# skyhehe123/SA-SSD

Measured on NVIDIA H100. Metric: KITTI frames/sec (~20k pts, car_cfg voxel grid), higher is better.
Workload: dtype f32

## Files before the change

include/sassd_b200.h:

```cpp
#ifndef SASSD_B200_H
#define SASSD_B200_H

#include <stddef.h>
#include <stdint.h>

#ifdef __cplusplus
extern "C" {
#endif

typedef void* sassd_stream_t;

enum {
    SASSD_OK = 0,
    SASSD_ERR_ARG = -1,
    SASSD_ERR_LAUNCH = -2,
    SASSD_ERR_WORKSPACE = -3,
    SASSD_ERR_UNSUPPORTED = -4
};

enum {
    SASSD_FLAG_VOXEL_CAP = 1,
    SASSD_FLAG_ROWS_CAP = 2,
    SASSD_FLAG_GUIDED_CAP = 4,
    SASSD_FLAG_NMS_CAP = 8,
// ... 68 lines not shown
typedef struct {
    int32_t mode, precision;
    int32_t cin, cout, taps;
    int32_t in_stride, out_stride;
    int32_t rows_cap;
    int32_t batch, H, W;
    int32_t relu;
} sassd_gconv_desc;
int sassd_gconv(const sassd_gconv_desc* host_desc, const float* in, const float* weight, const float* scale,
                const float* shift, const int32_t* nbr, const int32_t* d_rows, float* out, sassd_stream_t stream);

size_t sassd_gconv_pack_bytes(int taps, int cin, int cout, int precision);
int sassd_gconv_pack(const float* weight, int taps, int cin, int cout, int precision, void* packed,
                     sassd_stream_t stream);

typedef struct {
    int32_t batch, H, W;
    int32_t cin, cin_stored;
    int32_t cout, taps, relu;
    int32_t out_f32_stride, out_split_ch;
    int32_t tile_order;
    int32_t n_split;
} sassd_conv2d_desc;
int sassd_conv2d_f16x3(const sassd_conv2d_desc* host_desc, const void* in_split, const void* wpack, const float* scale,
                       const float* shift, float* out_f32, void* out_split, sassd_stream_t stream);
#define SASSD_CONV2D_TILE_H 8
#define SASSD_CONV2D_TILE_W 16
#define SASSD_TILE_DIST_MAX 9
int sassd_conv2d_f16x3_occ(const sassd_conv2d_desc* host_desc, const void* in_split, const void* wpack,
                           const float* scale, const float* shift, float* out_f32, void* out_split,
// ... 126 lines not shown
```

sa-ssd_b200/csrc/conv2d_tma.cu:

```cuda
#include <cuda.h>

#include <cstdlib>

#include "tc_common.cuh"

namespace tma {

using namespace tc;

constexpr int TILE_H = SASSD_CONV2D_TILE_H, TILE_W = SASSD_CONV2D_TILE_W;
constexpr int BKC = 64;
constexpr int kConstTile = 1 << 30;
constexpr int kBgTile = 1 << 29;
constexpr int CONS_WARPS = CONS_THREADS / 32;
constexpr int THREADS2 = CONS_THREADS + 32;
constexpr int W_LOAD = CONS_WARPS;

constexpr int A_ROWS = TILE_H + 2;
constexpr int A_PLANE_BYTES = A_ROWS * TILE_W * 128;
constexpr int A_STAGE_BYTES = 2 * A_PLANE_BYTES;
constexpr int A_STAGES = 2;

template <int BN>
struct Cfg2 {
    static constexpr int B_TILE_BYTES = BN * 128;
    static constexpr int B_STAGE_BYTES = 2 * B_TILE_BYTES;
    static constexpr int B_STAGES = (BN >= 128) ? 4 : 6;
    static constexpr int RING_BYTES = A_STAGES * A_STAGE_BYTES + B_STAGES * B_STAGE_BYTES;
    static constexpr int ORDER_CAP = 4608;
    static constexpr int SMEM_BYTES = RING_BYTES + 1024 + 256 + ORDER_CAP / 4 + ORDER_CAP * 2;
    static_assert(SMEM_BYTES <= 227 * 1024, "dynamic shared memory above the sm_90 limit");
};

__device__ __forceinline__ void tma_load_4d(uint32_t dst, const CUtensorMap* map, int c0, int c1, int c2, int c3,
                                            uint32_t bar) {
    asm volatile(
        "cp.async.bulk.tensor.4d.shared::cluster.global.tile.mbarrier::complete_tx::bytes [%0], [%1, {%2, %3, %4, %5}], [%6];"
        ::"r"(dst), "l"(map), "r"(c0), "r"(c1), "r"(c2), "r"(c3), "r"(bar)
        : "memory");
}

struct Conv2dArgs {
    const void* wpack;
// ... 82 lines not shown
                                                int nthreads) {
    if (!p.out_split || c0 >= p.out_split_ch) return;
    const int vpp = (p.out_split_ch - c0) >> 3;
    const size_t plane = (size_t)p.batch * p.H * p.W * p.out_split_ch;
    const uint4 zero = make_uint4(0u, 0u, 0u, 0u);
    for (int i = tid; i < TILE_H * TILE_W * vpp; i += nthreads) {
        const int pix = i / vpp;
        const int y = ty * TILE_H + pix / TILE_W, x = tx * TILE_W + pix % TILE_W;
        if (y >= p.H || x >= p.W) continue;
        __half* dst = p.out_split + (((size_t)b * p.H + y) * p.W + x) * p.out_split_ch + c0 + 8 * (i % vpp);
        *(uint4*)dst = zero;
        *(uint4*)(dst + plane) = zero;
    }
}

template <int BN>
__global__ void __launch_bounds__(THREADS2, 1)
conv2d_tma_kernel(const __grid_constant__ CUtensorMap amap, const Conv2dArgs p, const Background bg) {
    using C = Cfg2<BN>;
    extern __shared__ uint8_t smem_raw[];
    __shared__ int s_ncomp;
    __shared__ int s_walk[6];
    const uint32_t base = (smem_u32(smem_raw) + 1023u) & ~1023u;
    uint8_t* base_ptr = smem_raw + (base - smem_u32(smem_raw));
    const uint32_t b_ring = base + A_STAGES * A_STAGE_BYTES;
    const uint32_t bar_base = base + C::RING_BYTES;
    auto a_full = [&](int s) { return bar_base + 8u * s; };
    auto a_empty = [&](int s) { return bar_base + 8u * (A_STAGES + s); };
    auto b_full = [&](int s) { return bar_base + 8u * (2 * A_STAGES + s); };
    auto b_empty = [&](int s) { return bar_base + 8u * (2 * A_STAGES + C::B_STAGES + s); };

    pdl_launch_dependents();
    const int warp = __shfl_sync(0xffffffffu, (int)(threadIdx.x >> 5), 0), lane = threadIdx.x & 31;
    const int tiles_x = (p.W + TILE_W - 1) / TILE_W, tiles_y = (p.H + TILE_H - 1) / TILE_H;
// ... 11 lines not shown
        s_walk[0] = s_walk[1] = nunits;
        s_walk[2] = s_walk[4] = nunits + blockIdx.x;
        s_walk[3] = 1;
        s_walk[5] = blockIdx.x;
    }
    __syncthreads();
    pdl_wait();

    uint32_t* verdict = (uint32_t*)(base_ptr + C::RING_BYTES + 256);
    uint16_t* order = (uint16_t*)(verdict + 2 * (C::ORDER_CAP / 32));
    const bool small_map = p.tile_dist != nullptr && ntiles <= C::ORDER_CAP;
    const bool use_order = p.tile_order && small_map;
    if (small_map) {
        const int nslots = (ntiles + 31) / 32;
#pragma unroll 1
        for (int i0 = 4 * warp; i0 < nslots; i0 += 4 * (THREADS2 / 32)) {
            int dist[4];
#pragma unroll
            for (int e = 0; e < 4; ++e) {
                const int t = (i0 + e) * 32 + lane;
                dist[e] = t < ntiles ? __ldg(&p.tile_dist[t]) : 0;
            }
#pragma unroll
            for (int e = 0; e < 4; ++e) {
                const int t = (i0 + e) * 32 + lane;
                const int f = t < ntiles ? tile_skip_flag(p, bg, dist[e], (t / tiles_x) % tiles_y, t % tiles_x, tiles_y,
                                                          tiles_x) : 0;
                const uint32_t cst = __ballot_sync(0xffffffffu, f == kConstTile);
                const uint32_t bgm = __ballot_sync(0xffffffffu, f == kBgTile);
                if (lane == 0 && i0 + e < nslots) {
                    verdict[i0 + e] = cst;
// ... 45 lines not shown
            }
        }
        __syncthreads();
    }
    auto next_unit = [&](int k) -> int {
        if (k < s_walk[0]) { k += gridDim.x; return k < s_walk[0] ? k : s_walk[2]; }
        if (k < s_walk[1]) { k += s_walk[3]; return k < s_walk[1] ? k : s_walk[4]; }
        return k + gridDim.x;
    };
    auto tile_ref = [&](int k) -> int {
        if (small_map) { const int v = order[k]; return (v & 0x3fff) | ((v & 0xc000) << 15); }
        if (!p.tile_dist) return k;
        return k | tile_skip_flag(p, bg, __ldg(&p.tile_dist[k]), (k / tiles_x) % tiles_y, k % tiles_x, tiles_y, tiles_x);
    };

    if (warp == W_LOAD) {
        if (lane == 0) {
            int a_stage = 0, b_stage = 0;
            uint32_t a_phase = 0, b_phase = 0;
            const uint32_t a_bytes = 2u * (TILE_H + 2 * halo) * TILE_W * 128;
            for (int k = s_walk[5]; k < nunits; k = next_unit(k)) {
                const int ref = tile_ref(k / nsplit), half = k % nsplit;
                if (ref & (kConstTile | kBgTile)) continue;
                const int tile = ref;
                const int b = tile / (tiles_y * tiles_x);
                const int ty = (tile / tiles_x) % tiles_y, tx = tile % tiles_x;
                const int y0 = ty * TILE_H, x0 = tx * TILE_W;
                for (int col = 0; col < ncols; ++col) {
                    const int dx = col - halo;
                    for (int kc = 0; kc < kchunks; ++kc) {
                        mbar_wait(a_empty(a_stage), a_phase ^ 1u);
                        const uint32_t a_hi = base + a_stage * A_STAGE_BYTES;
                        mbar_expect_tx(a_full(a_stage), a_bytes);
                        tma_load_4d(a_hi, &amap, kc * BKC, x0 + dx, y0 - halo, b, a_full(a_stage));
                        tma_load_4d(a_hi + A_PLANE_BYTES, &amap, kc * BKC, x0 + dx, y0 - halo, p.batch + b, a_full(a_stage));
                        if (++a_stage == A_STAGES) { a_stage = 0; a_phase ^= 1u; }
                        for (int row = 0; row < nrows; ++row) {
                            const int t = row * ncols + col;
                            mbar_wait(b_empty(b_stage), b_phase ^ 1u);
                            const uint32_t b_dst = b_ring + b_stage * C::B_STAGE_BYTES;
                            mbar_expect_tx(b_full(b_stage), C::B_STAGE_BYTES);
                            const uint8_t* src = (const uint8_t*)p.wpack +
                                                 (size_t)(t * kchunks + kc) * (size_t)(2 * nsplit) * C::B_TILE_BYTES +
                                                 (size_t)half * C::B_TILE_BYTES;
                            constexpr uint32_t kPiece = (C::B_TILE_BYTES >= 8192) ? 8192u : (uint32_t)C::B_TILE_BYTES;
#pragma unroll 1
                            for (int part = 0; part < 2; ++part)
#pragma unroll 1
                                for (uint32_t o = 0; o < (uint32_t)C::B_TILE_BYTES; o += kPiece)
                                    bulk_g2s(b_dst + part * C::B_TILE_BYTES + o,
                                             src + (size_t)part * nsplit * C::B_TILE_BYTES + o, kPiece, b_full(b_stage));
                            if (++b_stage == C::B_STAGES) { b_stage = 0; b_phase ^= 1u; }
                        }
                    }
                }
            }
        }
        if (p.out_split && nsplit * BN < p.out_split_ch) {
            __syncwarp();
            for (int k = s_walk[5]; k < nunits; k = next_unit(k)) {
                if (k % nsplit != nsplit - 1) continue;
                const int tile = tile_ref(k / nsplit) & ~(kConstTile | kBgTile);
                zero_split_tail(p, tile / (tiles_y * tiles_x), (tile / tiles_x) % tiles_y, tile % tiles_x, nsplit * BN,
                                lane, 32);
            }
        }
    } else {
        const int wg = threadIdx.x >> 7, t = threadIdx.x & 127;
        const int rl0 = wg * 64 + (t >> 5) * 16 + ((t & 31) >> 2);
        const size_t plane = (size_t)p.batch * p.H * p.W * p.out_split_ch;
        float big[BN / 2], small[BN / 2];
        int a_stage = 0, b_stage = 0;
        uint32_t a_phase = 0, b_phase = 0;
        int computed = 0;
        for (int k = s_walk[5]; k < nunits; k = next_unit(k)) {
            const int ref = tile_ref(k / nsplit), n_off = (k % nsplit) * BN;
            const int tile = ref & ~(kConstTile | kBgTile);
            const bool const_tile = (ref & kConstTile) != 0;
            const int b = tile / (tiles_y * tiles_x);
            const int ty = (tile / tiles_x) % tiles_y, tx = tile % tiles_x;
            if (ref & kBgTile) continue;
            if (const_tile) {
                const int ncols = min(BN, p.out_split_ch - n_off);
                if (p.out_split && !p.out_f32 && (ncols == 64 || ncols == 128 || ncols == 256)) {
                    store_constant_unit<CONS_WARPS>(p, b, ty, tx, n_off, ncols, warp, lane);
                    continue;
                }
            } else {
                if (k % nsplit == 0) ++computed;
#pragma unroll
                for (int i = 0; i < BN / 2; ++i) { big[i] = 0.f; small[i] = 0.f; }
                int prev_b = -1, prev_a = -1, row = 0;
                for (int ch = 0; ch < nchunks; ++ch) {
                    if (row == 0) mbar_wait(a_full(a_stage), a_phase);
                    mbar_wait(b_full(b_stage), b_phase);
                    const uint32_t ah = base + a_stage * A_STAGE_BYTES + (uint32_t)(row * TILE_W + wg * 64) * 128u;
                    const uint32_t bh = b_ring + b_stage * C::B_STAGE_BYTES;
                    wgmma_fence();
                    mma_chunk_x3<1, BN>(big, small, ah, ah + A_PLANE_BYTES, bh, bh + C::B_TILE_BYTES);
                    wgmma_commit();
                    wgmma_wait<1>();
                    if (t == 0) {
                        if (prev_b >= 0) mbar_arrive(b_empty(prev_b));
                        if (prev_a >= 0) mbar_arrive(a_empty(prev_a));
                    }
                    prev_b = b_stage;
                    if (++b_stage == C::B_STAGES) { b_stage = 0; b_phase ^= 1u; }
                    prev_a = -1;
                    if (++row == nrows) {
                        row = 0;
                        prev_a = a_stage;
                        if (++a_stage == A_STAGES) { a_stage = 0; a_phase ^= 1u; }
                    }
                }
                wgmma_wait<0>();
                fence_regs<BN / 2>(big);
                fence_regs<BN / 2>(small);
                if (t == 0) {
                    if (prev_b >= 0) mbar_arrive(b_empty(prev_b));
                    if (prev_a >= 0) mbar_arrive(a_empty(prev_a));
                }
            }
#pragma unroll
            for (int j = 0; j < BN / 8; ++j) {
                const int n = n_off + 8 * j + 2 * (t & 3);
                float c0, c1, sc0 = 1.f, sc1 = 1.f, sh0 = 0.f, sh1 = 0.f;
                if (const_tile) {
                    c0 = n < p.cout ? __ldg(&p.cvec[n]) : 0.f;
                    c1 = n + 1 < p.cout ? __ldg(&p.cvec[n + 1]) : 0.f;
                } else {
                    if (p.scale && n < p.cout) sc0 = __ldg(&p.scale[n]);
                    if (p.scale && n + 1 < p.cout) sc1 = __ldg(&p.scale[n + 1]);
                    if (p.shift && n < p.cout) sh0 = __ldg(&p.shift[n]);
                    if (p.shift && n + 1 < p.cout) sh1 = __ldg(&p.shift[n + 1]);
                }
#pragma unroll
                for (int i = 0; i < 2; ++i) {
                    const int rl = rl0 + 8 * i;
                    const int y = ty * TILE_H + rl / TILE_W, x = tx * TILE_W + rl % TILE_W;
                    float o0 = c0, o1 = c1;
                    if (!const_tile) {
                        o0 = fmaf(__fadd_rn(big[4 * j + 2 * i], small[4 * j + 2 * i] * (1.f / kF16LoScale)), sc0, sh0);
                        o1 = fmaf(__fadd_rn(big[4 * j + 2 * i + 1], small[4 * j + 2 * i + 1] * (1.f / kF16LoScale)), sc1, sh1);
                        if (p.relu) { o0 = fmaxf(o0, 0.f); o1 = fmaxf(o1, 0.f); }
                        if (n >= p.cout) o0 = 0.f;
                        if (n + 1 >= p.cout) o1 = 0.f;
                    }
                    if (y >= p.H || x >= p.W) continue;
                    const size_t pix = ((size_t)b * p.H + y) * p.W + x;
                    if (p.out_f32 && n < p.out_f32_stride)
                        *(float2*)(p.out_f32 + pix * p.out_f32_stride + n) = make_float2(o0, o1);
                    if (p.out_split && n < p.out_split_ch) {
                        uint32_t h, l;
                        split_f16x2(o0, o1, h, l);
                        __half* dst = p.out_split + pix * p.out_split_ch + n;
                        *(uint32_t*)dst = h;
                        *(uint32_t*)(dst + plane) = l;
                    }
                }
            }
        }
        if (bg.split || bg.f32) {
            for (int k = s_walk[5]; k < nunits; k = next_unit(k)) {
                const int ref = tile_ref(k / nsplit);
                if (!(ref & kBgTile)) continue;
                const int tile = ref & ~kBgTile;
                copy_background_unit(p, bg, tile / (tiles_y * tiles_x), (tile / tiles_x) % tiles_y, tile % tiles_x,
                                     (k % nsplit) * BN, BN, threadIdx.x, CONS_THREADS);
            }
        }
        if (p.counters && threadIdx.x == 0) {
            if (computed) atomicAdd(&p.counters[0], computed);
// ... 20 lines not shown
    return fn;
}

template <int BN>
static int launch2(const CUtensorMap& map, const Conv2dArgs& a, const Background& bg, cudaStream_t stream) {
    using C = Cfg2<BN>;
    auto kern = conv2d_tma_kernel<BN>;
    static bool configured = false;
    if (!configured) {
        if (cudaFuncSetAttribute(kern, cudaFuncAttributeMaxDynamicSharedMemorySize, C::SMEM_BYTES) != cudaSuccess)
            return SASSD_ERR_LAUNCH;
        configured = true;
    }
    const int units = a.batch * sassd_div_up(a.H, TILE_H) * sassd_div_up(a.W, TILE_W) * a.nsplit;
    const int grid = units < sassd_num_sms() ? units : sassd_num_sms();
    if (launch_pdl(kern, dim3(grid), dim3(THREADS2), C::SMEM_BYTES, stream, map, a, bg) != cudaSuccess) return SASSD_ERR_LAUNCH;
    return sassd_check_launch();
}

}

extern "C" int sassd_conv2d_f16x3(const sassd_conv2d_desc* d, const void* in_split, const void* wpack,
                                  const float* scale, const float* shift, float* out_f32, void* out_split,
                                  sassd_stream_t stream_) {
    return sassd_conv2d_f16x3_occ_bg(d, in_split, wpack, scale, shift, out_f32, out_split, nullptr, 0, nullptr, nullptr,
                                     nullptr, nullptr, stream_);
}

extern "C" int sassd_conv2d_f16x3_occ(const sassd_conv2d_desc* d, const void* in_split, const void* wpack,
                                      const float* scale, const float* shift, float* out_f32, void* out_split,
                                      const int32_t* tile_dist, int reach, const float* const_out, int32_t* counters,
                                      sassd_stream_t stream_) {
    return sassd_conv2d_f16x3_occ_bg(d, in_split, wpack, scale, shift, out_f32, out_split, tile_dist, reach, const_out,
                                     nullptr, nullptr, counters, stream_);
// ... 81 lines not shown
```

sa-ssd_b200/csrc/tc_common.cuh:

```cuda
#pragma once
#include <cuda_fp16.h>

#include "common.cuh"

#include <cstdlib>
#include <utility>

namespace tc {

constexpr int BM = 128;
constexpr int BK = 32;
constexpr int A_TILE_BYTES = BM * 128;
constexpr int CONS_THREADS = 256;

__device__ __forceinline__ uint32_t smem_u32(const void* p) { return (uint32_t)__cvta_generic_to_shared(p); }

__device__ __forceinline__ void mbar_init(uint32_t bar, uint32_t count) {
    asm volatile("mbarrier.init.shared::cta.b64 [%0], %1;" ::"r"(bar), "r"(count));
}
__device__ __forceinline__ void mbar_arrive(uint32_t bar) {
    asm volatile("mbarrier.arrive.shared::cta.b64 _, [%0];" ::"r"(bar) : "memory");
}
__device__ __forceinline__ void mbar_expect_tx(uint32_t bar, uint32_t bytes) {
    asm volatile("mbarrier.arrive.expect_tx.shared::cta.b64 _, [%0], %1;" ::"r"(bar), "r"(bytes) : "memory");
// ... 97 lines not shown
template <>
__device__ __forceinline__ void wgmma<0, 64>(float (&d)[32], uint64_t da, uint64_t db, uint32_t scale_d) {
    asm volatile(
        "{\n\t.reg .pred p;\n\tsetp.ne.b32 p, %34, 0;\n\t"
        "wgmma.mma_async.sync.aligned.m64n64k8.f32.tf32.tf32 {%0, %1, %2, %3, %4, %5, %6, %7, %8, %9, %10, %11, %12, %13, %14, %15, %16, %17, %18, %19, %20, %21, %22, %23, %24, %25, %26, %27, %28, %29, %30, %31}, %32, %33, p, 1, 1;\n\t}\n"
        : "+f"(d[0]), "+f"(d[1]), "+f"(d[2]), "+f"(d[3]), "+f"(d[4]), "+f"(d[5]), "+f"(d[6]), "+f"(d[7]), "+f"(d[8]), "+f"(d[9]), "+f"(d[10]), "+f"(d[11]), "+f"(d[12]), "+f"(d[13]), "+f"(d[14]), "+f"(d[15]), "+f"(d[16]), "+f"(d[17]), "+f"(d[18]), "+f"(d[19]), "+f"(d[20]), "+f"(d[21]), "+f"(d[22]), "+f"(d[23]), "+f"(d[24]), "+f"(d[25]), "+f"(d[26]), "+f"(d[27]), "+f"(d[28]), "+f"(d[29]), "+f"(d[30]), "+f"(d[31])
        : "l"(da), "l"(db), "r"(scale_d) : "memory");
}
template <>
__device__ __forceinline__ void wgmma<0, 128>(float (&d)[64], uint64_t da, uint64_t db, uint32_t scale_d) {
    asm volatile(
        "{\n\t.reg .pred p;\n\tsetp.ne.b32 p, %66, 0;\n\t"
        "wgmma.mma_async.sync.aligned.m64n128k8.f32.tf32.tf32 {%0, %1, %2, %3, %4, %5, %6, %7, %8, %9, %10, %11, %12, %13, %14, %15, %16, %17, %18, %19, %20, %21, %22, %23, %24, %25, %26, %27, %28, %29, %30, %31, %32, %33, %34, %35, %36, %37, %38, %39, %40, %41, %42, %43, %44, %45, %46, %47, %48, %49, %50, %51, %52, %53, %54, %55, %56, %57, %58, %59, %60, %61, %62, %63}, %64, %65, p, 1, 1;\n\t}\n"
        : "+f"(d[0]), "+f"(d[1]), "+f"(d[2]), "+f"(d[3]), "+f"(d[4]), "+f"(d[5]), "+f"(d[6]), "+f"(d[7]), "+f"(d[8]), "+f"(d[9]), "+f"(d[10]), "+f"(d[11]), "+f"(d[12]), "+f"(d[13]), "+f"(d[14]), "+f"(d[15]), "+f"(d[16]), "+f"(d[17]), "+f"(d[18]), "+f"(d[19]), "+f"(d[20]), "+f"(d[21]), "+f"(d[22]), "+f"(d[23]), "+f"(d[24]), "+f"(d[25]), "+f"(d[26]), "+f"(d[27]), "+f"(d[28]), "+f"(d[29]), "+f"(d[30]), "+f"(d[31]), "+f"(d[32]), "+f"(d[33]), "+f"(d[34]), "+f"(d[35]), "+f"(d[36]), "+f"(d[37]), "+f"(d[38]), "+f"(d[39]), "+f"(d[40]), "+f"(d[41]), "+f"(d[42]), "+f"(d[43]), "+f"(d[44]), "+f"(d[45]), "+f"(d[46]), "+f"(d[47]), "+f"(d[48]), "+f"(d[49]), "+f"(d[50]), "+f"(d[51]), "+f"(d[52]), "+f"(d[53]), "+f"(d[54]), "+f"(d[55]), "+f"(d[56]), "+f"(d[57]), "+f"(d[58]), "+f"(d[59]), "+f"(d[60]), "+f"(d[61]), "+f"(d[62]), "+f"(d[63])
        : "l"(da), "l"(db), "r"(scale_d) : "memory");
}

template <int PREC, int N>
__device__ __forceinline__ void mma_chunk_x3(float (&big)[N / 2], float (&small)[N / 2], uint32_t a_hi, uint32_t a_lo,
                                             uint32_t b_hi, uint32_t b_lo, bool big_fresh = false) {
    const uint64_t dah = make_desc(a_hi), dal = make_desc(a_lo), dbh = make_desc(b_hi), dbl = make_desc(b_lo);
#pragma unroll
    for (int k = 0; k < 4; ++k) {
        const uint64_t ko = 2ull * (uint64_t)k;
        wgmma<PREC, N>(small, dal + ko, dbh + ko, 1u);
        wgmma<PREC, N>(small, dah + ko, dbl + ko, 1u);
        wgmma<PREC, N>(big, dah + ko, dbh + ko, (k == 0 && big_fresh) ? 0u : 1u);
    }
}

// ... 59 lines not shown
```

sa-ssd_b200/lib.py:

```python
import ctypes
import os

from . import build as _build

c_int, c_float, c_size_t, c_void_p = ctypes.c_int, ctypes.c_float, ctypes.c_size_t, ctypes.c_void_p


class VoxelParams(ctypes.Structure):
    _fields_ = [("voxel_size", c_float * 3), ("range_min", c_float * 3), ("grid", ctypes.c_int32 * 3),
                ("max_points", ctypes.c_int32), ("max_voxels", ctypes.c_int32)]


class Conv2dDesc(ctypes.Structure):
    _fields_ = [(n, ctypes.c_int32) for n in ("batch", "H", "W", "cin", "cin_stored", "cout", "taps", "relu",
                                              "out_f32_stride", "out_split_ch", "tile_order", "n_split")]


class SpconvDesc(ctypes.Structure):
    _fields_ = [(n, ctypes.c_int32) for n in ("cin", "cout", "taps", "rows_cap", "in_rows_cap", "relu", "out_ch",
                                              "out_f32_stride")]


class GConvDesc(ctypes.Structure):
    _fields_ = [(n, ctypes.c_int32) for n in ("mode", "precision", "cin", "cout", "taps", "in_stride", "out_stride",
# ... 39 lines not shown
                                       P]),
    "sassd_anchor_mask_workspace_bytes": (c_size_t, [c_int, c_int, c_int]),
    "sassd_anchor_mask": (c_int, [P, P, c_int, c_int, c_int, c_int, P, c_int, c_int, P, P, c_size_t, P]),
    "sassd_hash_build": (c_int, [P, P, c_int, c_int, c_int, c_int, c_int, P, P, c_int, P, P]),
    "sassd_rulebook_subm": (c_int, [P, P, c_int, c_int, c_int, c_int, P, P, c_int, P, P, P]),
    "sassd_rulebook_conv_workspace_bytes": (c_size_t, [c_int, c_int, c_int, c_int]),
    "sassd_rulebook_conv_outputs": (c_int, [P, P, c_int, c_int, c_int, c_int, c_int, P, P, c_int, P, P, c_size_t, P]),
    "sassd_set_pdl": (c_int, [c_int]),
    "sassd_rulebook_conv_outputs_hash": (c_int, [P, P, c_int, c_int, c_int, c_int, c_int, P, P, c_int, P, P, c_int, P, P,
                                                 c_size_t, P]),
    "sassd_rulebook_conv_nbr": (c_int, [P, P, c_int, c_int, c_int, c_int, P, P, c_int, P, P, P]),
    "sassd_rulebook_pairs": (c_int, [P, P, c_int, P, P, P]),
    "sassd_gconv": (c_int, [ctypes.POINTER(GConvDesc), P, P, P, P, P, P, P, P]),
    "sassd_gconv_pack_bytes": (c_size_t, [c_int, c_int, c_int, c_int]),
    "sassd_gconv_pack": (c_int, [P, c_int, c_int, c_int, c_int, P, P]),
    "sassd_conv2d_f16x3": (c_int, [ctypes.POINTER(Conv2dDesc), P, P, P, P, P, P, P]),
    "sassd_conv2d_f16x3_occ": (c_int, [ctypes.POINTER(Conv2dDesc), P, P, P, P, P, P, P, c_int, P, P, P]),
    "sassd_conv2d_f16x3_occ_bg": (c_int, [ctypes.POINTER(Conv2dDesc), P, P, P, P, P, P, P, c_int, P, P, P, P, P]),
    "sassd_rotate_overlap_eval": (c_int, [P, P, P, P, P, c_int, c_int, c_int, P, P]),
    "sassd_kitti_match": (c_int, [c_int, P, P, P, P, P, P, P, P, P, P, P, P, c_int, ctypes.c_double, c_int, c_int, P, P,
                                  P, P]),
    "sassd_spconv_pack_bytes": (c_size_t, [c_int, c_int, c_int]),
    "sassd_spconv_pack": (c_int, [P, c_int, c_int, c_int, c_int, P, P]),
    "sassd_spconv_workspace_bytes": (c_size_t, []),
    "sassd_spconv_f16x3": (c_int, [ctypes.POINTER(SpconvDesc), P, P, P, P, P, P, P, P, P, P, c_size_t, P, P]),
    "sassd_features_to_split": (c_int, [P, P, c_int, c_int, c_int, P, P]),
    "sassd_split_rows_to_bev": (c_int, [P, P, P, c_int, c_int, c_int, c_int, c_int, c_int, P, P, P]),
    "sassd_sparse_to_bev_split": (c_int, [P, P, P, c_int, c_int, c_int, c_int, c_int, c_int, P, P, P]),
    "sassd_sparse_to_bev": (c_int, [P, P, P, c_int, c_int, c_int, c_int, c_int, P, P]),
    "sassd_decode_select_workspace_bytes": (c_size_t, [c_int, c_int]),
# ... 69 lines not shown
```

sa-ssd_b200/ops.py:

```python
import collections
import ctypes
import os
import math

import numpy as np
import torch

from . import lib as _lib
from .lib import Conv2dDesc, SpconvDesc
from .lib import (GCONV_CONV2D, GCONV_ROWS, GCONV_TABLE, PREC_F16X3, PREC_FP32, PREC_TF32X3, GConvDesc, VoxelParams,
                  check)

NMS_CAP = 4096
DEFAULT_PRECISION = PREC_F16X3


def _L():
    return _lib.load()


def _stream():
    return ctypes.c_void_p(torch.cuda.current_stream().cuda_stream)


# ... 3 lines not shown
    assert t.is_cuda and t.is_contiguous(), "sassd ops need contiguous CUDA tensors"
    return ctypes.c_void_p(t.data_ptr())


def require_cuda():
    if not torch.cuda.is_available():
        raise _lib.SassdError("sassd_b200 needs a CUDA device (sm_90a); there is no CPU fallback")


def next_pow2(n):
    return 1 << max(1, int(math.ceil(math.log2(max(2, n)))))


_KERNELS = {"sassd_voxelize": 4, "sassd_voxel_mean": 1, "sassd_frustum_crop": 1, "sassd_image_fov_crop": 1, "sassd_points_in_rbboxes": 1, "sassd_augment_drop_points": 1, "sassd_augment_noise_search": 1, "sassd_augment_assemble": 1, "sassd_anchor_mask": 4, "sassd_hash_build": 1,
            "sassd_rulebook_subm": 1, "sassd_rulebook_conv_outputs": 2, "sassd_rulebook_conv_outputs_hash": 2, "sassd_rulebook_conv_nbr": 1,
            "sassd_rulebook_pairs": 1, "sassd_gconv": 1, "sassd_gconv_pack": 1, "sassd_spconv_pack": 1, "sassd_rotate_overlap_eval": 1, "sassd_conv2d_f16x3": 1, "sassd_conv2d_f16x3_occ": 1, "sassd_conv2d_f16x3_occ_bg": 1, "sassd_spconv_f16x3": 1, "sassd_features_to_split": 1, "sassd_split_rows_to_bev": 1, "sassd_sparse_to_bev_split": 1, "sassd_sparse_to_bev": 1, "sassd_decode_select": 2,
            "sassd_pswarp": 1, "sassd_rescore_nms": 3, "sassd_kitti_format": 1, "sassd_three_nn": 1, "sassd_point_aux_head": 1, "sassd_nms_mask": 1, "sassd_nms_sorted": 2,
            "sassd_boxes_iou_bev": 1, "sassd_points_in_boxes": 2, "sassd_assign_rpn": 3, "sassd_assign_pswarp": 3,
            "sassd_rpn_loss": 2, "sassd_pswarp_loss": 2, "sassd_aux_loss": 2}
LAUNCHES = 0
PROFILE = None


def _call(name, label, *args):
    global LAUNCHES
    LAUNCHES += _KERNELS[name]
    fn = getattr(_L(), name)
    if PROFILE is None:
        check(fn(*args), name)
        return
    e0 = torch.cuda.Event(enable_timing=True)
# ... 235 lines not shown
def pack_tc(weight, precision):
    taps, cin, cout = weight.shape
    nbytes = _L().sassd_gconv_pack_bytes(taps, cin, cout, precision)
    packed = torch.empty((nbytes,), dtype=torch.uint8, device=weight.device)
    _call("sassd_gconv_pack", None, _ptr(weight), taps, cin, cout, precision, _ptr(packed), _stream())
    return packed


def tc_pack_cached(weight, precision):
    key = (weight.data_ptr(), weight._version, tuple(weight.shape), precision)
    ent = _TC_PACKS.get(key)
    if ent is None:
        if len(_TC_PACKS) >= 256:
            _TC_PACKS.pop(next(iter(_TC_PACKS)))
        ent = (pack_tc(weight.contiguous(), precision), weight)
        _TC_PACKS[key] = ent
    return ent[0]


def spconv_pack_cached(weight, cin_stored):
    key = (weight.data_ptr(), weight._version, tuple(weight.shape), "spconv", cin_stored)
    ent = _TC_PACKS.get(key)
    if ent is None:
        if len(_TC_PACKS) >= 256:
            _TC_PACKS.pop(next(iter(_TC_PACKS)))
        w = weight.contiguous()
        taps, cin, cout = w.shape
        nbytes = _L().sassd_spconv_pack_bytes(taps, cin_stored, cout)
        if nbytes == 0:
            raise _lib.SassdError("sassd_spconv_pack_bytes: unsupported shape taps=%d cin_stored=%d cout=%d"
# ... 325 lines not shown
        BACKGROUND_PINS.append(ent[0])
    return ent[0]


def sparse_to_bev_split(feat, coors, d_rows, C, D, H, W, batch):
    planes = torch.zeros((2, batch, H, W, D * C), dtype=torch.float16, device=feat.device)
    dist = _tile_dist(batch, H, W, feat.device)
    _call("sassd_sparse_to_bev_split", None, _ptr(feat), _ptr(coors), _ptr(d_rows), feat.shape[0], C, D, H, W, batch,
          _ptr(planes), _ptr(dist), _stream())
    return SplitMap(planes, D * C, dist)


def conv2d_split(x, weight, scale, shift, relu, cout, out_split=True, out_f32=False):
    B, H, W, cin = x.shape
    taps = weight.shape[0]
    wp = tc_pack_cached(weight, PREC_F16X3)
    d = Conv2dDesc()
    d.batch, d.H, d.W, d.cin, d.cin_stored = B, H, W, cin, x.planes.shape[-1]
    d.cout, d.taps, d.relu = cout, taps, 1 if relu else 0
    d.tile_order = CONV2D_TILE_ORDER
    d.n_split = 0
    osp = of = None
    if out_split:
        cs = (cout + 63) // 64 * 64
        osp = torch.empty((2, B, H, W, cs), dtype=torch.float16, device=x.device)
        d.out_split_ch = cs
    if out_f32:
        stride = (cout + 3) // 4 * 4
        of = torch.empty((B, H, W, stride), dtype=torch.float32, device=x.device)
        d.out_f32_stride = stride
    label = "conv2d_tma[taps=%d %d->%d]" % (taps, cin, cout)
# ... 64 lines not shown
```

Measured before the change: 806.5.

## Use register-sourced wgmma with weights in registers for wide conv2d tiles

For BN>=128 the conv2d TMA kernel now treats the weights as the register-sourced A operand of wgmma (m64n128k16) and the activation tile as the shared-memory B operand, effectively transposing the GEMM. Weights are prepacked into per-thread fragment blocks and double-buffered through ld.global.nc, so the shared-memory weight ring and its mbarrier traffic go away and a third activation stage is added. Register reallocation via setmaxnreg gives the math warpgroups more registers, and the epilogue stages outputs through padded shared memory so global stores are coalesced. In exchange, weight loads now come straight from global/L2 on the critical path, register pressure is high, and a new packing format and pack kernel are required.

```diff
diff --git a/include/sassd_b200.h b/include/sassd_b200.h
--- a/include/sassd_b200.h
+++ b/include/sassd_b200.h
@@ -106,6 +106,8 @@
 int sassd_gconv_pack(const float* weight, int taps, int cin, int cout, int precision, void* packed,
                      sassd_stream_t stream);
 
+size_t sassd_conv2d_pack_bytes(int taps, int cin, int cout);
+int sassd_conv2d_pack(const float* weight, int taps, int cin, int cout, void* packed, sassd_stream_t stream);
 typedef struct {
     int32_t batch, H, W;
     int32_t cin, cin_stored;
diff --git a/sa-ssd_b200/csrc/conv2d_tma.cu b/sa-ssd_b200/csrc/conv2d_tma.cu
--- a/sa-ssd_b200/csrc/conv2d_tma.cu
+++ b/sa-ssd_b200/csrc/conv2d_tma.cu
@@ -13,20 +13,25 @@
 constexpr int kConstTile = 1 << 30;
 constexpr int kBgTile = 1 << 29;
 constexpr int CONS_WARPS = CONS_THREADS / 32;
-constexpr int THREADS2 = CONS_THREADS + 32;
 constexpr int W_LOAD = CONS_WARPS;
 
 constexpr int A_ROWS = TILE_H + 2;
 constexpr int A_PLANE_BYTES = A_ROWS * TILE_W * 128;
 constexpr int A_STAGE_BYTES = 2 * A_PLANE_BYTES;
-constexpr int A_STAGES = 2;
+
+constexpr int FRAG_BLOCK_BYTES = 128 * 32;
+constexpr int OUT_PITCH = 64 + 4;
 
 template <int BN>
 struct Cfg2 {
+    static constexpr bool RS = BN >= 128;
+    static constexpr int THREADS = CONS_THREADS + (RS ? 128 : 32);
+    static constexpr int A_STAGES = RS ? 3 : 2;
     static constexpr int B_TILE_BYTES = BN * 128;
     static constexpr int B_STAGE_BYTES = 2 * B_TILE_BYTES;
-    static constexpr int B_STAGES = (BN >= 128) ? 4 : 6;
-    static constexpr int RING_BYTES = A_STAGES * A_STAGE_BYTES + B_STAGES * B_STAGE_BYTES;
+    static constexpr int B_STAGES = RS ? 0 : 6;
+    static constexpr int OUT_BYTES = RS ? 2 * TILE_H * TILE_W * OUT_PITCH * 4 : 0;
+    static constexpr int RING_BYTES = A_STAGES * A_STAGE_BYTES + B_STAGES * B_STAGE_BYTES + OUT_BYTES;
     static constexpr int ORDER_CAP = 4608;
     static constexpr int SMEM_BYTES = RING_BYTES + 1024 + 256 + ORDER_CAP / 4 + ORDER_CAP * 2;
     static_assert(SMEM_BYTES <= 227 * 1024, "dynamic shared memory above the sm_90 limit");
@@ -139,10 +144,25 @@
     }
 }
 
+__device__ __forceinline__ void mma_chunk_x3_rs(float (&big)[64], float (&small)[64], const uint32_t (&w)[32],
+                                                uint32_t x_hi, uint32_t x_lo) {
+    const uint64_t dxh = make_desc(x_hi), dxl = make_desc(x_lo);
+#pragma unroll
+    for (int k = 0; k < 4; ++k) {
+        const uint64_t ko = 2ull * (uint64_t)k;
+        const uint32_t wh[4] = {w[8 * k], w[8 * k + 1], w[8 * k + 2], w[8 * k + 3]};
+        const uint32_t wl[4] = {w[8 * k + 4], w[8 * k + 5], w[8 * k + 6], w[8 * k + 7]};
+        wgmma_rs_n128(small, wh, dxl + ko);
+        wgmma_rs_n128(small, wl, dxh + ko);
+        wgmma_rs_n128(big, wh, dxh + ko);
+    }
+}
+
 template <int BN>
-__global__ void __launch_bounds__(THREADS2, 1)
+__global__ void __launch_bounds__(Cfg2<BN>::THREADS, 1)
 conv2d_tma_kernel(const __grid_constant__ CUtensorMap amap, const Conv2dArgs p, const Background bg) {
     using C = Cfg2<BN>;
+    constexpr int A_STAGES = C::A_STAGES;
     extern __shared__ uint8_t smem_raw[];
     __shared__ int s_ncomp;
     __shared__ int s_walk[6];
@@ -184,7 +204,7 @@
     if (small_map) {
         const int nslots = (ntiles + 31) / 32;
 #pragma unroll 1
-        for (int i0 = 4 * warp; i0 < nslots; i0 += 4 * (THREADS2 / 32)) {
+        for (int i0 = 4 * warp; i0 < nslots; i0 += 4 * (C::THREADS / 32)) {
             int dist[4];
 #pragma unroll
             for (int e = 0; e < 4; ++e) {
@@ -260,7 +280,11 @@
         return k | tile_skip_flag(p, bg, __ldg(&p.tile_dist[k]), (k / tiles_x) % tiles_y, k % tiles_x, tiles_y, tiles_x);
     };
 
-    if (warp == W_LOAD) {
+    if (warp >= W_LOAD) {
+        if constexpr (C::RS) {
+            setmaxnreg_dec<40>();
+            if (warp != W_LOAD) return;
+        }
         if (lane == 0) {
             int a_stage = 0, b_stage = 0;
             uint32_t a_phase = 0, b_phase = 0;
@@ -281,22 +305,24 @@
                         tma_load_4d(a_hi, &amap, kc * BKC, x0 + dx, y0 - halo, b, a_full(a_stage));
                         tma_load_4d(a_hi + A_PLANE_BYTES, &amap, kc * BKC, x0 + dx, y0 - halo, p.batch + b, a_full(a_stage));
                         if (++a_stage == A_STAGES) { a_stage = 0; a_phase ^= 1u; }
-                        for (int row = 0; row < nrows; ++row) {
-                            const int t = row * ncols + col;
-                            mbar_wait(b_empty(b_stage), b_phase ^ 1u);
-                            const uint32_t b_dst = b_ring + b_stage * C::B_STAGE_BYTES;
-                            mbar_expect_tx(b_full(b_stage), C::B_STAGE_BYTES);
-                            const uint8_t* src = (const uint8_t*)p.wpack +
-                                                 (size_t)(t * kchunks + kc) * (size_t)(2 * nsplit) * C::B_TILE_BYTES +
-                                                 (size_t)half * C::B_TILE_BYTES;
-                            constexpr uint32_t kPiece = (C::B_TILE_BYTES >= 8192) ? 8192u : (uint32_t)C::B_TILE_BYTES;
+                        if constexpr (!C::RS) {
+                            for (int row = 0; row < nrows; ++row) {
+                                const int t = row * ncols + col;
+                                mbar_wait(b_empty(b_stage), b_phase ^ 1u);
+                                const uint32_t b_dst = b_ring + b_stage * C::B_STAGE_BYTES;
+                                mbar_expect_tx(b_full(b_stage), C::B_STAGE_BYTES);
+                                const uint8_t* src = (const uint8_t*)p.wpack +
+                                                     (size_t)(t * kchunks + kc) * (size_t)(2 * nsplit) * C::B_TILE_BYTES +
+                                                     (size_t)half * C::B_TILE_BYTES;
+                                constexpr uint32_t kPiece = (C::B_TILE_BYTES >= 8192) ? 8192u : (uint32_t)C::B_TILE_BYTES;
 #pragma unroll 1
-                            for (int part = 0; part < 2; ++part)
+                                for (int part = 0; part < 2; ++part)
 #pragma unroll 1
-                                for (uint32_t o = 0; o < (uint32_t)C::B_TILE_BYTES; o += kPiece)
-                                    bulk_g2s(b_dst + part * C::B_TILE_BYTES + o,
-                                             src + (size_t)part * nsplit * C::B_TILE_BYTES + o, kPiece, b_full(b_stage));
-                            if (++b_stage == C::B_STAGES) { b_stage = 0; b_phase ^= 1u; }
+                                    for (uint32_t o = 0; o < (uint32_t)C::B_TILE_BYTES; o += kPiece)
+                                        bulk_g2s(b_dst + part * C::B_TILE_BYTES + o,
+                                                 src + (size_t)part * nsplit * C::B_TILE_BYTES + o, kPiece, b_full(b_stage));
+                                if (++b_stage == C::B_STAGES) { b_stage = 0; b_phase ^= 1u; }
+                            }
                         }
                     }
                 }
@@ -312,6 +338,7 @@
             }
         }
     } else {
+        if constexpr (C::RS) setmaxnreg_inc<232>();
         const int wg = threadIdx.x >> 7, t = threadIdx.x & 127;
         const int rl0 = wg * 64 + (t >> 5) * 16 + ((t & 31) >> 2);
         const size_t plane = (size_t)p.batch * p.H * p.W * p.out_split_ch;
@@ -337,26 +364,67 @@
 #pragma unroll
                 for (int i = 0; i < BN / 2; ++i) { big[i] = 0.f; small[i] = 0.f; }
                 int prev_b = -1, prev_a = -1, row = 0;
-                for (int ch = 0; ch < nchunks; ++ch) {
-                    if (row == 0) mbar_wait(a_full(a_stage), a_phase);
-                    mbar_wait(b_full(b_stage), b_phase);
-                    const uint32_t ah = base + a_stage * A_STAGE_BYTES + (uint32_t)(row * TILE_W + wg * 64) * 128u;
-                    const uint32_t bh = b_ring + b_stage * C::B_STAGE_BYTES;
-                    wgmma_fence();
-                    mma_chunk_x3<1, BN>(big, small, ah, ah + A_PLANE_BYTES, bh, bh + C::B_TILE_BYTES);
-                    wgmma_commit();
-                    wgmma_wait<1>();
-                    if (t == 0) {
-                        if (prev_b >= 0) mbar_arrive(b_empty(prev_b));
-                        if (prev_a >= 0) mbar_arrive(a_empty(prev_a));
+                if constexpr (C::RS) {
+                    const uint32_t kstep = 2u * nsplit * FRAG_BLOCK_BYTES, qstep = 4u * kstep;
+                    const uint8_t* wsrc = (const uint8_t*)p.wpack + (2 * (k % nsplit) + wg) * FRAG_BLOCK_BYTES + t * 32;
+                    auto load_w = [&](uint32_t (&w)[32], int q) {
+                        const uint8_t* src = wsrc + (size_t)q * qstep;
+#pragma unroll
+                        for (int s = 0; s < 4; ++s) {
+                            const uint4 h = ldg_nc_v4(src + s * kstep), l = ldg_nc_v4(src + s * kstep + 16);
+                            w[8 * s] = h.x; w[8 * s + 1] = h.y; w[8 * s + 2] = h.z; w[8 * s + 3] = h.w;
+                            w[8 * s + 4] = l.x; w[8 * s + 5] = l.y; w[8 * s + 6] = l.z; w[8 * s + 7] = l.w;
+                        }
+                    };
+                    auto chunk = [&](uint32_t (&w)[32], uint32_t (&w_next)[32], int ch) {
+                        if (row == 0) mbar_wait(a_full(a_stage), a_phase);
+                        const uint32_t xh = base + a_stage * A_STAGE_BYTES + (uint32_t)row * (TILE_W * 128u);
+                        wgmma_fence();
+                        mma_chunk_x3_rs(big, small, w, xh, xh + A_PLANE_BYTES);
+                        wgmma_commit();
+                        wgmma_wait<1>();
+                        fence_regs<32>(w_next);
+                        if (t == 0 && prev_a >= 0) mbar_arrive(a_empty(prev_a));
+                        if (ch + 1 < nchunks) load_w(w_next, ch + 1);
+                        prev_a = -1;
+                        if (++row == nrows) {
+                            row = 0;
+                            prev_a = a_stage;
+                            if (++a_stage == A_STAGES) { a_stage = 0; a_phase ^= 1u; }
+                        }
+                    };
+                    uint32_t wa[32], wb[32];
+                    load_w(wa, 0);
+                    for (int ch = 0; ch < nchunks; ch += 2) {
+                        chunk(wa, wb, ch);
+                        if (ch + 1 == nchunks) break;
+                        chunk(wb, wa, ch + 1);
                     }
-                    prev_b = b_stage;
-                    if (++b_stage == C::B_STAGES) { b_stage = 0; b_phase ^= 1u; }
-                    prev_a = -1;
-                    if (++row == nrows) {
-                        row = 0;
-                        prev_a = a_stage;
-                        if (++a_stage == A_STAGES) { a_stage = 0; a_phase ^= 1u; }
+                    wgmma_wait<0>();
+                    fence_regs<32>(wa);
+                    fence_regs<32>(wb);
+                } else {
+                    for (int ch = 0; ch < nchunks; ++ch) {
+                        if (row == 0) mbar_wait(a_full(a_stage), a_phase);
+                        mbar_wait(b_full(b_stage), b_phase);
+                        const uint32_t ah = base + a_stage * A_STAGE_BYTES + (uint32_t)(row * TILE_W + wg * 64) * 128u;
+                        const uint32_t bh = b_ring + b_stage * C::B_STAGE_BYTES;
+                        wgmma_fence();
+                        mma_chunk_x3<1, BN>(big, small, ah, ah + A_PLANE_BYTES, bh, bh + C::B_TILE_BYTES);
+                        wgmma_commit();
+                        wgmma_wait<1>();
+                        if (t == 0) {
+                            if (prev_b >= 0) mbar_arrive(b_empty(prev_b));
+                            if (prev_a >= 0) mbar_arrive(a_empty(prev_a));
+                        }
+                        prev_b = b_stage;
+                        if (++b_stage == C::B_STAGES) { b_stage = 0; b_phase ^= 1u; }
+                        prev_a = -1;
+                        if (++row == nrows) {
+                            row = 0;
+                            prev_a = a_stage;
+                            if (++a_stage == A_STAGES) { a_stage = 0; a_phase ^= 1u; }
+                        }
                     }
                 }
                 wgmma_wait<0>();
@@ -367,41 +435,97 @@
                     if (prev_a >= 0) mbar_arrive(a_empty(prev_a));
                 }
             }
-#pragma unroll
-            for (int j = 0; j < BN / 8; ++j) {
-                const int n = n_off + 8 * j + 2 * (t & 3);
-                float c0, c1, sc0 = 1.f, sc1 = 1.f, sh0 = 0.f, sh1 = 0.f;
-                if (const_tile) {
-                    c0 = n < p.cout ? __ldg(&p.cvec[n]) : 0.f;
-                    c1 = n + 1 < p.cout ? __ldg(&p.cvec[n + 1]) : 0.f;
-                } else {
-                    if (p.scale && n < p.cout) sc0 = __ldg(&p.scale[n]);
-                    if (p.scale && n + 1 < p.cout) sc1 = __ldg(&p.scale[n + 1]);
-                    if (p.shift && n < p.cout) sh0 = __ldg(&p.shift[n]);
-                    if (p.shift && n + 1 < p.cout) sh1 = __ldg(&p.shift[n + 1]);
-                }
+            if constexpr (C::RS) {
+                float* stage = (float*)(base_ptr + A_STAGES * A_STAGE_BYTES) + wg * (TILE_H * TILE_W * OUT_PITCH);
+                const int m0 = 16 * (t >> 5) + ((t & 31) >> 2), c_wg = n_off + 64 * wg;
+                float cv[2], sc[2], sh[2];
 #pragma unroll
                 for (int i = 0; i < 2; ++i) {
-                    const int rl = rl0 + 8 * i;
-                    const int y = ty * TILE_H + rl / TILE_W, x = tx * TILE_W + rl % TILE_W;
-                    float o0 = c0, o1 = c1;
-                    if (!const_tile) {
-                        o0 = fmaf(__fadd_rn(big[4 * j + 2 * i], small[4 * j + 2 * i] * (1.f / kF16LoScale)), sc0, sh0);
-                        o1 = fmaf(__fadd_rn(big[4 * j + 2 * i + 1], small[4 * j + 2 * i + 1] * (1.f / kF16LoScale)), sc1, sh1);
-                        if (p.relu) { o0 = fmaxf(o0, 0.f); o1 = fmaxf(o1, 0.f); }
-                        if (n >= p.cout) o0 = 0.f;
-                        if (n + 1 >= p.cout) o1 = 0.f;
+                    const int n = c_wg + m0 + 8 * i;
+                    cv[i] = const_tile && n < p.cout ? __ldg(&p.cvec[n]) : 0.f;
+                    sc[i] = p.scale && n < p.cout ? __ldg(&p.scale[n]) : 1.f;
+                    sh[i] = p.shift && n < p.cout ? __ldg(&p.shift[n]) : 0.f;
+                }
+                named_bar_sync(1 + wg, 128);
+#pragma unroll
+                for (int j = 0; j < 16; ++j)
+#pragma unroll
+                    for (int i = 0; i < 2; ++i)
+#pragma unroll
+                        for (int e = 0; e < 2; ++e) {
+                            float o = cv[i];
+                            if (!const_tile) {
+                                o = fmaf(__fadd_rn(big[4 * j + 2 * i + e], small[4 * j + 2 * i + e] * (1.f / kF16LoScale)),
+                                         sc[i], sh[i]);
+                                if (p.relu) o = fmaxf(o, 0.f);
+                                if (c_wg + m0 + 8 * i >= p.cout) o = 0.f;
+                            }
+                            stage[(8 * j + 2 * (t & 3) + e) * OUT_PITCH + m0 + 8 * i] = o;
+                        }
+                named_bar_sync(1 + wg, 128);
+                if (p.out_f32) {
+                    for (int v = t; v < TILE_H * TILE_W * 16; v += 128) {
+                        const int pix = v >> 4, c = 4 * (v & 15), n = c_wg + c;
+                        const int y = ty * TILE_H + pix / TILE_W, x = tx * TILE_W + pix % TILE_W;
+                        if (n >= p.out_f32_stride || y >= p.H || x >= p.W) continue;
+                        *(float4*)(p.out_f32 + (((size_t)b * p.H + y) * p.W + x) * p.out_f32_stride + n) =
+                            *(const float4*)(stage + pix * OUT_PITCH + c);
                     }
-                    if (y >= p.H || x >= p.W) continue;
-                    const size_t pix = ((size_t)b * p.H + y) * p.W + x;
-                    if (p.out_f32 && n < p.out_f32_stride)
-                        *(float2*)(p.out_f32 + pix * p.out_f32_stride + n) = make_float2(o0, o1);
-                    if (p.out_split && n < p.out_split_ch) {
-                        uint32_t h, l;
-                        split_f16x2(o0, o1, h, l);
-                        __half* dst = p.out_split + pix * p.out_split_ch + n;
-                        *(uint32_t*)dst = h;
-                        *(uint32_t*)(dst + plane) = l;
+                }
+                if (p.out_split) {
+                    for (int v = t; v < TILE_H * TILE_W * 8; v += 128) {
+                        const int pix = v >> 3, c = 8 * (v & 7), n = c_wg + c;
+                        const int y = ty * TILE_H + pix / TILE_W, x = tx * TILE_W + pix % TILE_W;
+                        if (n >= p.out_split_ch || y >= p.H || x >= p.W) continue;
+                        const float4 f0 = *(const float4*)(stage + pix * OUT_PITCH + c);
+                        const float4 f1 = *(const float4*)(stage + pix * OUT_PITCH + c + 4);
+                        uint4 hi, lo;
+                        split_f16x2(f0.x, f0.y, hi.x, lo.x);
+                        split_f16x2(f0.z, f0.w, hi.y, lo.y);
+                        split_f16x2(f1.x, f1.y, hi.z, lo.z);
+                        split_f16x2(f1.z, f1.w, hi.w, lo.w);
+                        __half* dst = p.out_split + (((size_t)b * p.H + y) * p.W + x) * p.out_split_ch + n;
+                        *(uint4*)dst = hi;
+                        *(uint4*)(dst + plane) = lo;
+                    }
+                }
+            } else {
+#pragma unroll
+                for (int j = 0; j < BN / 8; ++j) {
+                    const int n = n_off + 8 * j + 2 * (t & 3);
+                    float c0, c1, sc0 = 1.f, sc1 = 1.f, sh0 = 0.f, sh1 = 0.f;
+                    if (const_tile) {
+                        c0 = n < p.cout ? __ldg(&p.cvec[n]) : 0.f;
+                        c1 = n + 1 < p.cout ? __ldg(&p.cvec[n + 1]) : 0.f;
+                    } else {
+                        if (p.scale && n < p.cout) sc0 = __ldg(&p.scale[n]);
+                        if (p.scale && n + 1 < p.cout) sc1 = __ldg(&p.scale[n + 1]);
+                        if (p.shift && n < p.cout) sh0 = __ldg(&p.shift[n]);
+                        if (p.shift && n + 1 < p.cout) sh1 = __ldg(&p.shift[n + 1]);
+                    }
+#pragma unroll
+                    for (int i = 0; i < 2; ++i) {
+                        const int rl = rl0 + 8 * i;
+                        const int y = ty * TILE_H + rl / TILE_W, x = tx * TILE_W + rl % TILE_W;
+                        float o0 = c0, o1 = c1;
+                        if (!const_tile) {
+                            o0 = fmaf(__fadd_rn(big[4 * j + 2 * i], small[4 * j + 2 * i] * (1.f / kF16LoScale)), sc0, sh0);
+                            o1 = fmaf(__fadd_rn(big[4 * j + 2 * i + 1], small[4 * j + 2 * i + 1] * (1.f / kF16LoScale)), sc1, sh1);
+                            if (p.relu) { o0 = fmaxf(o0, 0.f); o1 = fmaxf(o1, 0.f); }
+                            if (n >= p.cout) o0 = 0.f;
+                            if (n + 1 >= p.cout) o1 = 0.f;
+                        }
+                        if (y >= p.H || x >= p.W) continue;
+                        const size_t pix = ((size_t)b * p.H + y) * p.W + x;
+                        if (p.out_f32 && n < p.out_f32_stride)
+                            *(float2*)(p.out_f32 + pix * p.out_f32_stride + n) = make_float2(o0, o1);
+                        if (p.out_split && n < p.out_split_ch) {
+                            uint32_t h, l;
+                            split_f16x2(o0, o1, h, l);
+                            __half* dst = p.out_split + pix * p.out_split_ch + n;
+                            *(uint32_t*)dst = h;
+                            *(uint32_t*)(dst + plane) = l;
+                        }
                     }
                 }
             }
@@ -452,10 +576,51 @@
     }
     const int units = a.batch * sassd_div_up(a.H, TILE_H) * sassd_div_up(a.W, TILE_W) * a.nsplit;
     const int grid = units < sassd_num_sms() ? units : sassd_num_sms();
-    if (launch_pdl(kern, dim3(grid), dim3(THREADS2), C::SMEM_BYTES, stream, map, a, bg) != cudaSuccess) return SASSD_ERR_LAUNCH;
+    if (launch_pdl(kern, dim3(grid), dim3(C::THREADS), C::SMEM_BYTES, stream, map, a, bg) != cudaSuccess) return SASSD_ERR_LAUNCH;
     return sassd_check_launch();
 }
 
+__global__ void conv2d_pack_kernel(const float* __restrict__ w, int taps, int cin, int cout, int nblk,
+                                   uint32_t* __restrict__ out) {
+    const int kchunks = (cin + BKC - 1) / BKC, ncols = taps == 9 ? 3 : 1, nrows = ncols;
+    const long long total = (long long)taps * kchunks * 4 * nblk * (FRAG_BLOCK_BYTES / 4);
+    for (long long i = blockIdx.x * (long long)blockDim.x + threadIdx.x; i < total; i += (long long)gridDim.x * blockDim.x) {
+        const int word = (int)(i % 8), t = (int)((i / 8) % 128);
+        long long r = i / (FRAG_BLOCK_BYTES / 4);
+        const int mb = (int)(r % nblk);
+        r /= nblk;
+        const int s = (int)(r % 4), q = (int)(r / 4);
+        const int row = q % nrows, kc = (q / nrows) % kchunks, col = q / (nrows * kchunks);
+        const int tap = row * ncols + col, a = word % 4, lane = t % 32;
+        const int n = 64 * mb + 16 * (t / 32) + lane / 4 + 8 * (a & 1);
+        const int k = kc * BKC + 16 * s + 2 * (lane % 4) + 8 * (a >> 1);
+        float hi[2], lo[2];
+#pragma unroll
+        for (int e = 0; e < 2; ++e) {
+            const float v = (k + e < cin && n < cout) ? w[((size_t)tap * cin + k + e) * cout + n] : 0.f;
+            split_f16(v, hi[e], lo[e]);
+        }
+        const __half2 h = word < 4 ? __floats2half2_rn(hi[0], hi[1]) : __floats2half2_rn(lo[0], lo[1]);
+        out[i] = *reinterpret_cast<const uint32_t*>(&h);
+    }
+}
+
+}
+
+extern "C" size_t sassd_conv2d_pack_bytes(int taps, int cin, int cout) {
+    if (!(taps == 9 || taps == 1) || cin < 1 || cout < 1 || cout > 256) return 0;
+    if (cout <= 64) return sassd_gconv_pack_bytes(taps, cin, cout, SASSD_PREC_F16X3);
+    return (size_t)taps * ((cin + tma::BKC - 1) / tma::BKC) * 4 * (cout <= 128 ? 2 : 4) * tma::FRAG_BLOCK_BYTES;
+}
+
+extern "C" int sassd_conv2d_pack(const float* weight, int taps, int cin, int cout, void* packed,
+                                 sassd_stream_t stream_) {
+    if (!weight || !packed || sassd_conv2d_pack_bytes(taps, cin, cout) == 0) return SASSD_ERR_ARG;
+    if (cout <= 64) return sassd_gconv_pack(weight, taps, cin, cout, SASSD_PREC_F16X3, packed, stream_);
+    const long long words = (long long)sassd_conv2d_pack_bytes(taps, cin, cout) / 4;
+    tma::conv2d_pack_kernel<<<sassd_grid(words, 256), 256, 0, (cudaStream_t)stream_>>>(
+        weight, taps, cin, cout, cout <= 128 ? 2 : 4, (uint32_t*)packed);
+    return sassd_check_launch();
 }
 
 extern "C" int sassd_conv2d_f16x3(const sassd_conv2d_desc* d, const void* in_split, const void* wpack,
diff --git a/sa-ssd_b200/csrc/tc_common.cuh b/sa-ssd_b200/csrc/tc_common.cuh
--- a/sa-ssd_b200/csrc/tc_common.cuh
+++ b/sa-ssd_b200/csrc/tc_common.cuh
@@ -135,6 +135,31 @@
         "wgmma.mma_async.sync.aligned.m64n128k8.f32.tf32.tf32 {%0, %1, %2, %3, %4, %5, %6, %7, %8, %9, %10, %11, %12, %13, %14, %15, %16, %17, %18, %19, %20, %21, %22, %23, %24, %25, %26, %27, %28, %29, %30, %31, %32, %33, %34, %35, %36, %37, %38, %39, %40, %41, %42, %43, %44, %45, %46, %47, %48, %49, %50, %51, %52, %53, %54, %55, %56, %57, %58, %59, %60, %61, %62, %63}, %64, %65, p, 1, 1;\n\t}\n"
         : "+f"(d[0]), "+f"(d[1]), "+f"(d[2]), "+f"(d[3]), "+f"(d[4]), "+f"(d[5]), "+f"(d[6]), "+f"(d[7]), "+f"(d[8]), "+f"(d[9]), "+f"(d[10]), "+f"(d[11]), "+f"(d[12]), "+f"(d[13]), "+f"(d[14]), "+f"(d[15]), "+f"(d[16]), "+f"(d[17]), "+f"(d[18]), "+f"(d[19]), "+f"(d[20]), "+f"(d[21]), "+f"(d[22]), "+f"(d[23]), "+f"(d[24]), "+f"(d[25]), "+f"(d[26]), "+f"(d[27]), "+f"(d[28]), "+f"(d[29]), "+f"(d[30]), "+f"(d[31]), "+f"(d[32]), "+f"(d[33]), "+f"(d[34]), "+f"(d[35]), "+f"(d[36]), "+f"(d[37]), "+f"(d[38]), "+f"(d[39]), "+f"(d[40]), "+f"(d[41]), "+f"(d[42]), "+f"(d[43]), "+f"(d[44]), "+f"(d[45]), "+f"(d[46]), "+f"(d[47]), "+f"(d[48]), "+f"(d[49]), "+f"(d[50]), "+f"(d[51]), "+f"(d[52]), "+f"(d[53]), "+f"(d[54]), "+f"(d[55]), "+f"(d[56]), "+f"(d[57]), "+f"(d[58]), "+f"(d[59]), "+f"(d[60]), "+f"(d[61]), "+f"(d[62]), "+f"(d[63])
         : "l"(da), "l"(db), "r"(scale_d) : "memory");
+}
+
+__device__ __forceinline__ void wgmma_rs_n128(float (&d)[64], const uint32_t (&a)[4], uint64_t db) {
+    asm volatile(
+        "{\n\t.reg .pred p;\n\tsetp.ne.b32 p, 1, 0;\n\t"
+        "wgmma.mma_async.sync.aligned.m64n128k16.f32.f16.f16 {%0, %1, %2, %3, %4, %5, %6, %7, %8, %9, %10, %11, %12, %13, %14, %15, %16, %17, %18, %19, %20, %21, %22, %23, %24, %25, %26, %27, %28, %29, %30, %31, %32, %33, %34, %35, %36, %37, %38, %39, %40, %41, %42, %43, %44, %45, %46, %47, %48, %49, %50, %51, %52, %53, %54, %55, %56, %57, %58, %59, %60, %61, %62, %63}, {%64, %65, %66, %67}, %68, p, 1, 1, 0;\n\t}\n"
+        : "+f"(d[0]), "+f"(d[1]), "+f"(d[2]), "+f"(d[3]), "+f"(d[4]), "+f"(d[5]), "+f"(d[6]), "+f"(d[7]), "+f"(d[8]), "+f"(d[9]), "+f"(d[10]), "+f"(d[11]), "+f"(d[12]), "+f"(d[13]), "+f"(d[14]), "+f"(d[15]), "+f"(d[16]), "+f"(d[17]), "+f"(d[18]), "+f"(d[19]), "+f"(d[20]), "+f"(d[21]), "+f"(d[22]), "+f"(d[23]), "+f"(d[24]), "+f"(d[25]), "+f"(d[26]), "+f"(d[27]), "+f"(d[28]), "+f"(d[29]), "+f"(d[30]), "+f"(d[31]), "+f"(d[32]), "+f"(d[33]), "+f"(d[34]), "+f"(d[35]), "+f"(d[36]), "+f"(d[37]), "+f"(d[38]), "+f"(d[39]), "+f"(d[40]), "+f"(d[41]), "+f"(d[42]), "+f"(d[43]), "+f"(d[44]), "+f"(d[45]), "+f"(d[46]), "+f"(d[47]), "+f"(d[48]), "+f"(d[49]), "+f"(d[50]), "+f"(d[51]), "+f"(d[52]), "+f"(d[53]), "+f"(d[54]), "+f"(d[55]), "+f"(d[56]), "+f"(d[57]), "+f"(d[58]), "+f"(d[59]), "+f"(d[60]), "+f"(d[61]), "+f"(d[62]), "+f"(d[63])
+        : "r"(a[0]), "r"(a[1]), "r"(a[2]), "r"(a[3]), "l"(db) : "memory");
+}
+template <int R>
+__device__ __forceinline__ void fence_regs(uint32_t (&r)[R]) {
+#pragma unroll
+    for (int i = 0; i < R; ++i) asm volatile("" : "+r"(r[i])::"memory");
+}
+template <int N>
+__device__ __forceinline__ void setmaxnreg_dec() { asm volatile("setmaxnreg.dec.sync.aligned.u32 %0;" ::"n"(N)); }
+template <int N>
+__device__ __forceinline__ void setmaxnreg_inc() { asm volatile("setmaxnreg.inc.sync.aligned.u32 %0;" ::"n"(N)); }
+__device__ __forceinline__ void named_bar_sync(int id, int nthreads) {
+    asm volatile("bar.sync %0, %1;" ::"r"(id), "r"(nthreads) : "memory");
+}
+__device__ __forceinline__ uint4 ldg_nc_v4(const void* p) {
+    uint4 v;
+    asm volatile("ld.global.nc.v4.u32 {%0, %1, %2, %3}, [%4];" : "=r"(v.x), "=r"(v.y), "=r"(v.z), "=r"(v.w) : "l"(p));
+    return v;
 }
 
 template <int PREC, int N>
diff --git a/sa-ssd_b200/lib.py b/sa-ssd_b200/lib.py
--- a/sa-ssd_b200/lib.py
+++ b/sa-ssd_b200/lib.py
@@ -77,6 +77,8 @@
     "sassd_gconv": (c_int, [ctypes.POINTER(GConvDesc), P, P, P, P, P, P, P, P]),
     "sassd_gconv_pack_bytes": (c_size_t, [c_int, c_int, c_int, c_int]),
     "sassd_gconv_pack": (c_int, [P, c_int, c_int, c_int, c_int, P, P]),
+    "sassd_conv2d_pack_bytes": (c_size_t, [c_int, c_int, c_int]),
+    "sassd_conv2d_pack": (c_int, [P, c_int, c_int, c_int, P, P]),
     "sassd_conv2d_f16x3": (c_int, [ctypes.POINTER(Conv2dDesc), P, P, P, P, P, P, P]),
     "sassd_conv2d_f16x3_occ": (c_int, [ctypes.POINTER(Conv2dDesc), P, P, P, P, P, P, P, c_int, P, P, P]),
     "sassd_conv2d_f16x3_occ_bg": (c_int, [ctypes.POINTER(Conv2dDesc), P, P, P, P, P, P, P, c_int, P, P, P, P, P]),
diff --git a/sa-ssd_b200/ops.py b/sa-ssd_b200/ops.py
--- a/sa-ssd_b200/ops.py
+++ b/sa-ssd_b200/ops.py
@@ -41,7 +41,7 @@
 
 _KERNELS = {"sassd_voxelize": 4, "sassd_voxel_mean": 1, "sassd_frustum_crop": 1, "sassd_image_fov_crop": 1, "sassd_points_in_rbboxes": 1, "sassd_augment_drop_points": 1, "sassd_augment_noise_search": 1, "sassd_augment_assemble": 1, "sassd_anchor_mask": 4, "sassd_hash_build": 1,
             "sassd_rulebook_subm": 1, "sassd_rulebook_conv_outputs": 2, "sassd_rulebook_conv_outputs_hash": 2, "sassd_rulebook_conv_nbr": 1,
-            "sassd_rulebook_pairs": 1, "sassd_gconv": 1, "sassd_gconv_pack": 1, "sassd_spconv_pack": 1, "sassd_rotate_overlap_eval": 1, "sassd_conv2d_f16x3": 1, "sassd_conv2d_f16x3_occ": 1, "sassd_conv2d_f16x3_occ_bg": 1, "sassd_spconv_f16x3": 1, "sassd_features_to_split": 1, "sassd_split_rows_to_bev": 1, "sassd_sparse_to_bev_split": 1, "sassd_sparse_to_bev": 1, "sassd_decode_select": 2,
+            "sassd_rulebook_pairs": 1, "sassd_gconv": 1, "sassd_gconv_pack": 1, "sassd_spconv_pack": 1, "sassd_rotate_overlap_eval": 1, "sassd_conv2d_pack": 1, "sassd_conv2d_f16x3": 1, "sassd_conv2d_f16x3_occ": 1, "sassd_conv2d_f16x3_occ_bg": 1, "sassd_spconv_f16x3": 1, "sassd_features_to_split": 1, "sassd_split_rows_to_bev": 1, "sassd_sparse_to_bev_split": 1, "sassd_sparse_to_bev": 1, "sassd_decode_select": 2,
             "sassd_pswarp": 1, "sassd_rescore_nms": 3, "sassd_kitti_format": 1, "sassd_three_nn": 1, "sassd_point_aux_head": 1, "sassd_nms_mask": 1, "sassd_nms_sorted": 2,
             "sassd_boxes_iou_bev": 1, "sassd_points_in_boxes": 2, "sassd_assign_rpn": 3, "sassd_assign_pswarp": 3,
             "sassd_rpn_loss": 2, "sassd_pswarp_loss": 2, "sassd_aux_loss": 2}
@@ -307,6 +307,24 @@
         if len(_TC_PACKS) >= 256:
             _TC_PACKS.pop(next(iter(_TC_PACKS)))
         ent = (pack_tc(weight.contiguous(), precision), weight)
+        _TC_PACKS[key] = ent
+    return ent[0]
+
+
+def conv2d_pack_cached(weight):
+    key = (weight.data_ptr(), weight._version, tuple(weight.shape), "conv2d")
+    ent = _TC_PACKS.get(key)
+    if ent is None:
+        if len(_TC_PACKS) >= 256:
+            _TC_PACKS.pop(next(iter(_TC_PACKS)))
+        w = weight.contiguous()
+        taps, cin, cout = w.shape
+        nbytes = _L().sassd_conv2d_pack_bytes(taps, cin, cout)
+        if nbytes == 0:
+            raise _lib.SassdError("sassd_conv2d_pack_bytes: unsupported shape taps=%d cin=%d cout=%d" % (taps, cin, cout))
+        packed = torch.empty((nbytes,), dtype=torch.uint8, device=w.device)
+        _call("sassd_conv2d_pack", None, _ptr(w), taps, cin, cout, _ptr(packed), _stream())
+        ent = (packed, weight)
         _TC_PACKS[key] = ent
     return ent[0]
 
@@ -662,7 +680,7 @@
 def conv2d_split(x, weight, scale, shift, relu, cout, out_split=True, out_f32=False):
     B, H, W, cin = x.shape
     taps = weight.shape[0]
-    wp = tc_pack_cached(weight, PREC_F16X3)
+    wp = conv2d_pack_cached(weight)
     d = Conv2dDesc()
     d.batch, d.H, d.W, d.cin, d.cin_stored = B, H, W, cin, x.planes.shape[-1]
     d.cout, d.taps, d.relu = cout, taps, 1 if relu else 0
```

Result: faster. 873.0 (median of 6 runs) (+8.3%).
